# Simple-Robotics/LoIK

Hardware: AMD Instinct MI355X
Metric: IK solves/sec to 1e-6 residual, Talos humanoid, batch=65536 per GPU (higher is better)
Workload: dtype f64

## Files before the change

### loik_amd/csrc/loik_device.hpp

```cpp
#pragma once

#include <hip/hip_runtime.h>

namespace loikb {

constexpr int WAVE = 64;

enum : int {
  JP_CS = 0,
  JP_V = 1,
  JP_F = 4,
  JP_G = 7,
  JP_WZ = 10,
  JP_NUS = 11,
  JP_P = 12,
  JP_R = 15,
  JP_LBUB = 16,
  JP_UD = 17,
  JREC = 20,
  JP_NPERSIST = 12,
  CP_Y = 0,
  CP_ATY = 3,
  CP_B = 6,
  CP_ATB = 9,
// ... 1589 lines not shown
        }
    }
    for (int i = 0; i < 6; ++i) {
      T a = T(0);
      for (int k = 0; k < 6; ++k) a += Al[6 * k + i] * bl[k];
      *elem_ptr<T>(crec, CP_ATB + i / 2, i & 1) = a;
    }
  }
  *elem_ptr<T>(srec, SP_BI, 0) = bn;
}

template <typename T>
__global__ void k_edit_constraints(char* tiles, Layout L, int c_lo, int c_hi, int shift, int B)
{
  const int b = blockIdx.x * blockDim.x + threadIdx.x;
  if (b >= B) return;
  char* lp = lane_ptr<T>(tiles, L, b);
  for (int c = c_lo; c < c_hi; ++c) {
    char* dst = lp + (size_t)(L.off_c + c * L.crec) * pair_bytes<T>();
    const char* src = dst + (size_t)L.crec * pair_bytes<T>();
    const bool copy = shift && c + 1 < c_hi;
    for (int k = 0; k < L.crec; ++k)
      for (int h = 0; h < 2; ++h) *elem_ptr<T>(dst, k, h) = copy ? *elem_ptr<T>(const_cast<char*>(src), k, h) : T(0);
  }
}

enum : int {
  RS_DATA_COLD = 1,
  RS_RECURSION = 2,
  RS_SOLVER = 4,
  RS_Y = 8,
  RS_HCACHE = 16,
  RS_MU = 32,
};
template <typename T>
__device__ __forceinline__ void reset_tile(char* tiles, const Layout& L, int what, T mu0, int tile, int lane)
{
  char* lp = tiles + (size_t)tile * L.tile_pairs * pair_bytes<T>() + (size_t)lane * 2 * sizeof(T);
  if (what & (RS_DATA_COLD | RS_RECURSION)) {
    for (int j = 0; j < L.nb; ++j) {
      char* rec = lp + (size_t)j * JREC * pair_bytes<T>();
      for (int p = JP_V; p < JP_WZ; ++p) stp<T>(rec, p, T(0), T(0));
      stp<T>(rec, JP_WZ, T(0), T(0));
      if (what & RS_DATA_COLD) st_lo<T>(rec, JP_NUS, T(0));
    }
  }
  if (what & (RS_RECURSION | RS_Y)) {
    for (int c = 0; c < L.nc; ++c) {
      char* crec = lp + (size_t)(L.off_c + c * L.crec) * pair_bytes<T>();
      for (int p = CP_Y; p < CP_B; ++p) stp<T>(crec, p, T(0), T(0));
    }
  }
  char* srec = lp + (size_t)L.off_s * pair_bytes<T>();
  if (what & RS_SOLVER) {
    stp<T>(srec, SP_MU, mu0, T(0));
    st_hi<T>(srec, SP_BI, T(0));
    stp<T>(srec, SP_ST, T(0), T(0));
    for (int p = SP_SCAL; p < SREC; ++p) stp<T>(srec, p, T(0), T(0));
  }
  if (what & RS_SOLVER) stp<T>(srec, SP_FLIP, T(0), T(0));
  if (what & RS_MU) stp<T>(srec, SP_MU, mu0, T(0));
  if (what & RS_HCACHE) stp<T>(srec, SP_TAG, T(-1), T(0));
}
template <typename T>
__global__ void __launch_bounds__(WAVE) k_reset(char* tiles, Layout L, int what, T mu0)
{
  reset_tile<T>(tiles, L, what, mu0, (int)blockIdx.x, (int)threadIdx.x);
}

struct MovePlan {
  char* src;
  char* dst_live;
// ... 51 lines not shown
```

### loik_amd/csrc/loik_flat.hpp

```cpp
#pragma once

#include "loik_lean.hpp"

namespace loikb {

constexpr int FLAT_RED = 8;
constexpr int FLAT_PART = 8;
constexpr int FLAT_JMP = 5;
constexpr int FLAT_MAXA = 16;
constexpr int FOLDW = 10;
constexpr int FLAT_COUNTERS_SLOT_HITS = 12;
constexpr int FLAT_NA_SMALL = 10;
constexpr int FSLOT_ROWS = 8;

struct FlatLane {
  int depth;
  int size;
  int jmp[FLAT_JMP];
  int anc[FLAT_MAXA];
  int red[FLAT_RED];
  int helper;
  int part[FLAT_PART];
};

enum : int { FC_LANE = 0, FC_B = 1, FC_Y = 7, FC_ATY = 13, FC_ATYW = 19, FC_ATBW = 25, FC_DY = 31, FC_DLT = 37, FC_ATYF = 43, FC_AW = 49, FC_A = 85,
              FC_VC = FC_DLT , FCD = 121 };
enum : int { FI_BNORM = 0, FI_TGIN, FI_STY, FI_TOLP, FI_TOLD, FI_DYQP, FI_ATDY, FI_UBP, FI_LBM, FI_C1, FI_C2, FI_PRIMAL, FI_DUAL, FI_DX,
             FI_DZ, FI_MULAST, FI_RED , FISC = FI_RED + 16 };

template <int NA>
__host__ __device__ constexpr int flat_xregion()
{
  int n = XROWS * 9;
  if (NA * WAVE + 2 > n) n = NA * WAVE + 2;
  if (WAVE * FOLDW > n) n = WAVE * FOLDW;
  return (n + 1) & ~1;
}
template <int NA> __host__ __device__ constexpr int flat_off_wl() { return flat_xregion<NA>(); }
template <int NA> __host__ __device__ constexpr int flat_off_nbuf() { return flat_off_wl<NA>() + 2 * (NA + 1) * WAVE; }
template <int NA> __host__ __device__ constexpr int flat_off_pbuf() { return flat_off_nbuf<NA>() + WAVE + 2; }
template <int NA> __host__ __device__ constexpr int flat_off_rbuf() { return flat_off_pbuf<NA>() + WAVE + 2; }
template <int NA> __host__ __device__ constexpr int flat_off_tail() { return flat_off_rbuf<NA>() + WAVE; }

template <typename T, int NA>
__host__ __device__ __forceinline__ size_t flat_lds_bytes(int nc, int G, bool a_shared, bool has_hv)
// ... 979 lines not shown
        }
      }
      tail_sync();
      if (on) {
        const T mu = mutab[dsl];
        const T mu_eq = P.mu_scale * mu, mu_in = mu;
        if (cslot >= 0) {
          const T* at = ata_l + (sub * L.nc + cslot) * 21;
#pragma unroll
          for (int k = 0; k < 21; ++k) hh[k] += mu_eq * at[k];
        }
        T U[6], UD[6];
        symv(hh, Sw, U);
        const T dinv = T(1) / (dot6_halves(Sw, U) + mu_in);
#pragma unroll
        for (int k = 0; k < 6; ++k) UD[k] = U[k] * dinv;
#pragma unroll
        for (int k = 0; k < 6; ++k) fslots[fslotA_at(sidx, ndec, dsl, frows, G, k, jlane)] = UD[k];
        fslots[fslotA_at(sidx, ndec, dsl, frows, G, 6, jlane)] = dinv;
        if (has_parent) {
          T* x = xch + lane * HX;
#pragma unroll
          for (int a = 0; a < 6; ++a)
#pragma unroll
            for (int b2 = a; b2 < 6; ++b2) x[sym(a, b2)] = hh[sym(a, b2)] - UD[a] * U[b2];
        }
      }
      tail_sync();
    }
  }
  lb[NA * WAVE + lane] = T(0);
  __builtin_amdgcn_s_waitcnt(0);
  tail_sync();
  for (int dsl = dw0; dsl < dw0 + nw; ++dsl) {
    T UDw[6], dinv = T(0);
#pragma unroll
    for (int k = 0; k < 6; ++k) UDw[k] = isj ? fslots[fslotA_at(sidx, ndec, dsl, frows, G, k, jlane)] : T(0);
    if (isj) dinv = fslots[fslotA_at(sidx, ndec, dsl, frows, G, 6, jlane)];
    T Lc[NA], Wc[NA];
#pragma unroll
    for (int k = 0; k < NA; ++k) {
      Lc[k] = dot6_halves(swt + arow[k] * 6, UDw);
      Wc[k] = T(0);
    }
    tail_sync();
#pragma unroll
    for (int k = 0; k < NA; ++k) lb[k * WAVE + lane] = Lc[k];
    tail_sync();
#pragma unroll
    for (int k = NA - 1; k >= 0; --k) {
      T acc = Lc[k];
#pragma unroll
      for (int k2 = k + 1; k2 < NA; ++k2) acc += lb[k * WAVE + arow[k2]] * Wc[k2];
      Wc[k] = (k < depth - 1) ? -acc : T(0);
    }
    tail_sync();
    if (isj) {
      const size_t base = fslotW_at(sidx, ndec, dsl, frows, fcol);
#pragma unroll
      for (int k = 0; k < NA; ++k)
        if (k < depth - 1) fslots[base + k] = Wc[k];
      fslots[base + depth - 1] = dinv;
    }
  }
}

template <typename T>
__global__ void k_rebuild_ud(char* tiles, Layout L, const JointDesc* __restrict__ jd, const T* __restrict__ uni, T rho, T mu_scale,
                             const T* __restrict__ href_tab, int a_shared, int B, T* __restrict__ scratch)
{
  const int b = blockIdx.x * blockDim.x + threadIdx.x;
  if (b >= B) return;
  char* lp = lane_ptr<T>(tiles, L, b);
  char* srec = lp + (size_t)L.off_s * pair_bytes<T>();
  if (*elem_ptr<T>(srec, SP_TAG, 0) != T(-2)) return;
  const T mu = *elem_ptr<T>(srec, SP_ST, 1);
  const T mu_eq = mu_scale * mu, mu_in = mu;
  T* o = scratch + (size_t)b * L.nb * 21;
  for (int i = 1; i <= L.nb; ++i) {
    for (int r = 0; r < 6; ++r)
      for (int c = r; c < 6; ++c)
        o[(i - 1) * 21 + sym(r, c)] = (jd[i].flags & JF_MASSLESS) ? T(0) : ((r == c ? rho : T(0)) + href_tab[(size_t)i * HREF_ROW + 6 * r + c]);
    if (jd[i].cslot >= 0) {
      const int cs = jd[i].cslot;
      for (int k = 0; k < 21; ++k) {
        const T a = a_shared ? uni[L.nc * 36 + cs * 21 + k]
                             : *elem_ptr<T>(lp + (size_t)(L.off_c + cs * L.crec) * pair_bytes<T>(), CP_ATA + k / 2, k & 1);
        o[(i - 1) * 21 + k] += mu_eq * a;
      }
    }
  }
  for (int i = L.nb; i >= 1; --i) {
    const JointDesc d = jd[i];
    T hh[21], U[6], UD[6], R[9], t[3], part[21];
    for (int k = 0; k < 21; ++k) hh[k] = o[(i - 1) * 21 + k];
// ... 36 lines not shown
```

### loik_amd/csrc/loik_host.hip

```cpp
#include "loik_device.hpp"
#include "loik_tail.hpp"
#include "loik_lean.hpp"
#include "loik_flat.hpp"
#include "loik_flat2.hpp"
#include "loik_passes.hpp"
#include "loik_pose.hpp"
#include "loik_pose_tasks.hpp"
#include "loik_pose_multistart.hpp"
#include "loik_pose_path.hpp"
#include "loik_pose_track.hpp"
#include "loik_pose_accel.hpp"
#include "loik_pose_step.hpp"
#include "loik_flat_inst.hpp"
#ifdef LOIKB_FLAT_SEPARATE_TU
LOIKB_FLAT2_INSTANCES(LOIKB_FLAT2_DECL)
LOIKB_FLAT1_INSTANCES(LOIKB_FLAT1_DECL)
#ifdef LOIKB_TAIL_PROF
int loikb_flat_prof_read(unsigned long long* out, int which, int reset);
#endif
#endif

#include "../../include/loik_amd.h"
#include "../../include/loik_amd_pose.h"
#include "../../include/loik_amd_limits.h"
// ... 213 lines not shown
    int* d_order = nullptr;
    unsigned int* d_order_bins = nullptr;
    int order_n = 0;
    unsigned long long order_epoch = 0;
    int order_holdoff = 0;
    int arrival_n = 0;
    double arrival_ms = 0.0;
    int* d_ring = nullptr;
    int ring_cap = 0;
    void* d_hslots = nullptr;
    size_t hslots_bytes = 0;
    void* d_fslots = nullptr;
    size_t fslots_bytes = 0;
    void* d_park = nullptr;
    unsigned int* d_fmask = nullptr;
    size_t fmask_n = 0;
    void** d_aux = nullptr;
    const void* aux_h[4] = {nullptr, nullptr, nullptr, nullptr};
    size_t park_bytes = 0;
    std::vector<int> h_wave;
    loikb_stats stats{};
    bool unfinished_counted = false;
    bool queue_ready = false;
    bool small_finished = false;
    int rc = 0;
    std::string err;
    std::vector<std::pair<float, float>> solve_iv, tail_iv;
  };
  std::vector<Chunk> chunks;
  hipEvent_t ev_fork = nullptr;
  loikb_stats stats{};
  bool pass_active = false;
  bool zero_state = false;
  unsigned long long inputs_epoch = 1;
  bool href_known = false;
  bool tab_bcast = false;
  double tab_H[36] = {0}, tab_v[6] = {0};
  int log_truncated = 0;
  PassLayout PL{};
  double* d_pass = nullptr;
  int* d_pass_cslot = nullptr;
  int seen_lo = 1 << 20, seen_hi = -(1 << 20);
  unsigned long long end_hist[32] = {0}, end_hist_n = 0;
  unsigned long long solve_serial = 0, end_hist_epoch = 0;
  double* d_log = nullptr;
  int* d_log_rows = nullptr;
  int log_rows_cap = 0;
  bool have_log = false;
  struct PoseState {
    double* d_tgt = nullptr;
    double* d_b = nullptr;
    double* d_err = nullptr;
    double* d_A = nullptr;
    int* d_status = nullptr;
    int* d_steps = nullptr;
    int* d_clink = nullptr;
    unsigned int* d_count = nullptr;
    int nc = 0;
    double timing[4] = {0, 0, 0, 0};
    bool have_limits = false;
    bool flags_valid = false;
    std::vector<PoseLimit> lim;
    PoseLimit* d_lim = nullptr;
    int* d_lflags = nullptr;
    unsigned char* d_inrange = nullptr;
    double2* d_box = nullptr;
// ... 1451 lines not shown
         !(S->opt.flags & (LOIKB_OPT_NO_COMPACTION | LOIKB_OPT_NO_H_CACHE)) && n <= tail_max && S->tune.direct_tail;
}

static bool bushy_goes_on_chip(const loikb_solver_impl* S)
{
  return direct_tail_of(S, S->B, std::max(1, batch_tail_max(S)));
}

template <typename T>
struct TailCtx {
  loikb_solver_impl* S; Chunk* C; Params<T>& P; Bufs<T> Bf;
  loikb_solver_impl::Set& A; int cur, n_cur;
  bool whole_set, small_flat;
  int G, ipw;
  int ndec, kexp_lo;
  const int* list; int n;
  double total_ms = 0.0;
  unsigned long long iters = 0;
};

struct OrderUse { bool ordered = false, was_stale = false; };

static int take_up_order(const loikb_solver_impl* S, Chunk* C, bool eligible, bool count_down, int n_cur, OrderUse* use)
{
  use->ordered = eligible && order_usable(S, C, n_cur);
  use->was_stale = use->ordered && C->order_epoch != S->inputs_epoch;
  if (count_down && C->order_holdoff > 0) --C->order_holdoff;
  if (use->ordered) HIPCHK(hipMemcpyAsync(C->d_slots, C->d_order, sizeof(int) * (size_t)n_cur, hipMemcpyDeviceToDevice, C->stream));
  C->stats.flat_ordered += use->ordered ? 1 : 0;
  return LOIKB_OK;
}

template <typename T>
static int leave_order(const loikb_solver_impl* S, Chunk* C, const loikb_solver_impl::Set& A, int n_cur, bool flat_engine)
{
  HIPCHK(hipMemsetAsync(C->d_order_bins, 0, sizeof(unsigned int) * 2 * ORDER_BINS, C->stream));
  hipLaunchKernelGGL(k_order_count<T>, grid1(n_cur), dim3(256), 0, C->stream, A.tiles, S->L, n_cur, S->opt.max_iter, C->d_order_bins,
                     flat_engine ? C->d_counters + ORDER_DEC_HIST : (unsigned int*)nullptr);
  if (flat_engine) HIPCHK(hipMemcpyAsync(C->h_counters, C->d_counters, NCOUNTERS * sizeof(unsigned int), hipMemcpyDeviceToHost, C->stream));
  hipLaunchKernelGGL(k_order_scan, dim3(1), dim3(ORDER_BINS), 0, C->stream, C->d_order_bins);
  hipLaunchKernelGGL(k_order_scatter<T>, grid1(n_cur), dim3(256), 0, C->stream, A.tiles, S->L, n_cur, S->opt.max_iter, C->d_order_bins, C->d_order);
  HIPCHK(hipGetLastError());
  C->order_n = n_cur;
  C->order_epoch = S->inputs_epoch;
  return LOIKB_OK;
}

static void judge_order(const loikb_solver_impl* S, Chunk* C, int n_cur, OrderUse use, double ms)
{
  if (C->arrival_n != n_cur) { C->arrival_n = n_cur; C->arrival_ms = 0.0; }
  if (!use.ordered) C->arrival_ms = ms;
  else if (use.was_stale && C->arrival_ms > 0.0 && ms > 0.985 * C->arrival_ms) C->order_holdoff = S->tune.flat_order_holdoff;
}

static void record_decades(loikb_solver_impl* S, unsigned int seen, int kexp_lo, unsigned int escaped)
{
  for (int d = 0; d < 16; ++d)
    if (seen & (1u << d)) { S->seen_lo = std::min(S->seen_lo, kexp_lo + d); S->seen_hi = std::max(S->seen_hi, kexp_lo + d); }
  if (escaped) { S->seen_lo = S->plan.kexp_lo; S->seen_hi = S->plan.kexp_lo + S->plan.ndec - 1; }
}

struct FlatLaunch {
  FlatKind kind; int nanc, frows, has_hv; bool small_na;
  int mur;
  int ndec, kexp_lo, dw0, nw;
  int slice;
  double cu_sh; dim3 grid;
};

static int flat_launch_slice(const loikb_solver_impl* S, const Chunk* C, FlatKind kind, int mur, int n, int n_cur, bool ordered)
{
  if (kind == FlatKind::Flat) return 0;
  if (kind == FlatKind::Flat1) return mur == 1 ? 0 : flat_slice_for(S, n, ordered);
  int q = flat_slice_for(S, n, ordered);
  if (q > 0 && (C->d_park == nullptr || (size_t)n_cur * flat2_park_stride(S->nc, true) * sizeof(double) > C->park_bytes)) q = 0;
  if (mur == 1 && S->tune.flat_slice < 0) q = 0;
  return q;
}

static void flat_table_window(const loikb_solver_impl* S, FlatLaunch& F, int n)
{
  int wlo = 0, whi = -1;
  const bool win_ok = F.slice > 0;
  if (S->tune.flat_win_n > 0) { wlo = S->tune.flat_win_lo; whi = wlo + S->tune.flat_win_n - 1; }
  else if (S->tune.flat_build == 2 && win_ok && S->end_hist_n > 0) {
    unsigned long long cum = 0;
    int k03 = 99, k97 = 99;
    for (int k = 0; k < 32; ++k) {
      cum += S->end_hist[k];
      if (k03 == 99 && cum * 100 >= 3ull * S->end_hist_n) k03 = k - 16;
      if (k97 == 99 && cum * 100 >= 97ull * S->end_hist_n) k97 = k - 16;
    }
    wlo = std::min(0, k03); whi = std::max(0, k97);
  }
// ... 97 lines not shown
  if (one_per_wave(F.kind) && X.whole_set && n_first == n_cur) judge_order(S, C, n_cur, use, (double)ms - (double)hms);
  if (S->tune.trace)
    fprintf(stderr, "[loikb] flat engine: %6d instances on %u workgroups, done at %8.3f ms (slots %6.3f ms)  "
                    "inst-iters %9u  wave-iters %7u  slot loads %7u (+ %u served from LDS)  escaped %u  still iterating %u\n",
            n_first, F.grid.x, ms, hms, C->h_counters[1], C->h_counters[5], C->h_counters[6],
            C->h_counters[FLAT_COUNTERS_SLOT_HITS], escaped, C->h_counters[3]);
  C->stats.lean_escaped += (int)escaped;
  C->tail_iv.emplace_back(t0, t0 + ms);
  X.total_ms = ms; X.n = (int)C->h_counters[3]; X.list = next;
  if (X.n == 0 && X.whole_set && X.cur == 0 && n_first == n_cur && S->chunks.size() == 1) { C->stats.n_unfinished = (int)C->h_counters[4]; C->unfinished_counted = true; C->small_finished = small_finish; }
  return LOIKB_OK;
}

template <typename T>
static int launch_flat(TailCtx<T>& X)
{
  loikb_solver_impl* S = X.S; Chunk* C = X.C;
  Params<T>& P = X.P;
  const int n = X.n, n_cur = X.n_cur;
  const bool small_flat = X.small_flat, whole_set = X.whole_set;
  FlatLaunch F;
  F.kind = flat_kind(S); F.nanc = S->flat.nanc; F.small_na = F.nanc <= FLAT_NA_SMALL; F.has_hv = S->Hv_inf_norm != 0.0;
  F.frows = S->flat.fblk;
  F.cu_sh = std::max(1.0, S->ncu * ((double)C->B / (double)S->B));
  F.ndec = X.ndec; F.kexp_lo = X.kexp_lo; F.dw0 = 0;
  const bool can_build2 = S->tune.flat_build && F.kind == FlatKind::Flat2 && C->d_fmask != nullptr && !S->opt.logging && !S->per_link && href_is_scalar(S);
  F.mur = flat_any_mu(S) ? 1 : (can_build2 ? 2 : 0);
  if (F.mur == 1) { F.ndec = 1; F.kexp_lo = 0; }
  if (F.mur == 2) { F.ndec = S->plan.ndec; F.kexp_lo = S->plan.kexp_lo; }
  const size_t need = (size_t)n_cur * F.ndec * F.frows * sizeof(T);
  if (need > C->fslots_bytes) { g_last_error = "internal: decade-slot buffer of the flat engine smaller than the chunk"; return LOIKB_ERR_STATE; }
  P.max_launch_iters = S->opt.max_iter + 1;
  const int mode_keep = P.mode;
  if (whole_set && S->zero_state && S->tune.flat_zero_state) P.mode |= MODE_ZERO_STATE;
  const bool queue_ready = small_flat && C->queue_ready && n_cur == S->B;
  C->queue_ready = false;
  if (!queue_ready && small_flat) hipLaunchKernelGGL(k_queue_init_iota, grid1(std::max(C->ring_cap, NCOUNTERS)), dim3(256), 0, C->stream, C->d_ring, C->ring_cap, C->d_slots, n_cur, C->d_counters, NCOUNTERS);
  else if (!queue_ready) HIPCHK(hipMemsetAsync(C->d_counters, 0, NCOUNTERS * sizeof(unsigned int), C->stream));
  if (!queue_ready) HIPCHK(hipEventRecord(C->ev_k0, C->stream));
  OrderUse use;
  int rc = take_up_order(S, C, !small_flat && whole_set && X.list == C->d_slots && n == n_cur && one_per_wave(F.kind), true, n_cur, &use);
  if (rc) return rc;
  F.slice = flat_launch_slice(S, C, F.kind, F.mur, n, n_cur, use.ordered);
  F.nw = F.ndec;
  if (F.mur == 2) flat_table_window(S, F, n);
  if (F.mur == 0) { F.ndec = X.ndec; F.kexp_lo = X.kexp_lo; F.nw = F.ndec; F.dw0 = 0; }
  if (F.ndec > 0) {
    const dim3 hgrid((unsigned)((n + X.ipw - 1) / X.ipw));
    const size_t slds = (std::max((size_t)(WAVE + 1) * 22, (size_t)((F.small_na ? FLAT_NA_SMALL : FLAT_MAXA) + 1) * WAVE) + (size_t)(WAVE + 1) * 6 +
                         (size_t)X.ipw * S->nc * 21 + 16) * sizeof(T);
    auto* fslots = F.small_na ? k_fslots<T, FLAT_NA_SMALL> : k_fslots<T, FLAT_MAXA>;
    hipLaunchKernelGGL(fslots, hgrid, dim3(WAVE), slds, C->stream, P, X.Bf, (const JointDesc*)S->d_jd, (const TailTopo*)S->d_topo,
                       (const int*)S->d_child_list, (const FlatLane*)S->flat.d_lanes, S->maxdepth, F.nanc, F.frows, S->flat.njmp, X.list, n,
                       X.G, (T*)C->d_fslots, F.kexp_lo, F.ndec, F.dw0, F.nw, F.mur == 2 ? C->d_fmask : (unsigned int*)nullptr);
    HIPCHK(hipGetLastError());
  }
  if (!small_flat) HIPCHK(hipEventRecord(C->ev_k2, C->stream));
  if (!small_flat) hipLaunchKernelGGL(k_ring_fill, grid1(C->ring_cap), dim3(256), 0, C->stream, C->d_ring, C->ring_cap, X.list, n, C->d_counters);
  if ((rc = launch_flat_kernel(X, F))) return rc;
  P.mode = mode_keep;
  int* next = (X.list == C->d_slots) ? C->d_slots2 : C->d_slots;
  const bool small_finish = small_flat && S->tune.small_finish;
  if (small_finish)
    hipLaunchKernelGGL(k_small_finish<T>, dim3(1), dim3(256), 0, C->stream, X.A.tiles, S->L, X.list, n, next, C->d_counters, NCOUNTERS, C->h_counters);
  else
    hipLaunchKernelGGL(k_list_unfinished<T>, grid1(n), dim3(256), 0, C->stream, X.A.tiles, S->L, X.list, n, next, C->d_counters + 3);
  HIPCHK(hipGetLastError());
  C->stats.launches++; C->stats.tail_launches++; C->stats.lean_launches++; C->stats.flat_launches++;
  if (F.kind == FlatKind::Flat2) C->stats.flat_split_launches++;
  HIPCHK(hipEventRecord(C->ev_k1, C->stream));
  const bool order_pass = !small_flat && S->tune.flat_order && whole_set && n == n_cur && one_per_wave(F.kind) && !(S->opt.flags & LOIKB_OPT_FIXED_ITERS);
  if (!order_pass && !small_finish) HIPCHK(hipMemcpyAsync(C->h_counters, C->d_counters, NCOUNTERS * sizeof(unsigned int), hipMemcpyDeviceToHost, C->stream));
  if (order_pass && (rc = leave_order<T>(S, C, X.A, n_cur, true))) return rc;
  HIPCHK(hipStreamSynchronize(C->stream));
  return flat_read_back(X, F, use, order_pass, small_finish, queue_ready, next);
}

template <typename T>
static int launch_lean(TailCtx<T>& X)
{
  loikb_solver_impl* S = X.S; Chunk* C = X.C;
  Params<T>& P = X.P;
  const Bufs<T>& Bf = X.Bf;
  const int n = X.n, n_cur = X.n_cur, G = X.G, ipw = X.ipw, ndec = X.ndec, kexp_lo = X.kexp_lo;
  const int* list = X.list;
  const bool whole_set = X.whole_set, per_link = S->per_link;
  const size_t need = (size_t)n_cur * ndec * HSLOT_PAIRS * G * 2 * sizeof(T);
  if (need > C->hslots_bytes) { g_last_error = "internal: decade-slot buffer smaller than the chunk"; return LOIKB_ERR_STATE; }
  const int waves_cu = S->plan.lean_waves_cu;
  const int ltw = S->plan.lean_wg_waves;
  const size_t lds = ltw * lean_lds_bytes<T>(S->nc, G, S->a_shared);
  if (lds > 64 * 1024) {
    HIPCHK(hipFuncSetAttribute((const void*)k_lean<T, true>, hipFuncAttributeMaxDynamicSharedMemorySize, (int)lds));
    HIPCHK(hipFuncSetAttribute((const void*)k_lean<T, false>, hipFuncAttributeMaxDynamicSharedMemorySize, (int)lds));
    HIPCHK(hipFuncSetAttribute((const void*)k_lean<T, false, true>, hipFuncAttributeMaxDynamicSharedMemorySize, (int)lds));
  }
  const int wg_per_cu = S->tune.lean_wg_per_cu > 0 ? S->tune.lean_wg_per_cu : waves_cu / ltw;
  const int wg_cap = wg_per_cu * std::max(1, (int)(S->ncu * ((double)C->B / (double)S->B) + 0.5));
  HIPCHK(hipEventRecord(C->ev_k0, C->stream));
  OrderUse use;
  int rc = take_up_order(S, C, whole_set && list == C->d_slots && n == n_cur, whole_set, n_cur, &use);
  if (rc) return rc;
  P.max_launch_iters = S->opt.max_iter + 1;
  const int wg_needed = (n + ipw * ltw - 1) / (ipw * ltw);
  const dim3 grid((unsigned)std::min(wg_needed, wg_cap));
  HIPCHK(hipMemsetAsync(C->d_counters, 0, NCOUNTERS * sizeof(unsigned int), C->stream));
// ... 93 lines not shown
  if (whole_set && !small_flat) {
    hipLaunchKernelGGL(k_list_iota, grid1(n_cur), dim3(256), 0, C->stream, C->d_slots, n_cur);
  } else if (!whole_set) {
    C->h_wave.resize(2 * (size_t)nw + 2);
    int* cnt = C->h_wave.data();
    int* off = cnt + nw + 1;
    HIPCHK(hipMemcpyAsync(cnt, A.wave_live, sizeof(int) * nw, hipMemcpyDeviceToHost, C->stream));
    HIPCHK(hipStreamSynchronize(C->stream));
    int total = 0;
    for (int w = 0; w < nw; ++w) { off[w] = total; total += cnt[w]; }
    if (total != n_live) { g_last_error = "tail: live count mismatch"; return LOIKB_ERR_STATE; }
    HIPCHK(hipMemcpyAsync(A.wave_off, off, sizeof(int) * nw, hipMemcpyHostToDevice, C->stream));
    hipLaunchKernelGGL(k_list_live<T>, dim3(nw), dim3(WAVE), 0, C->stream, A.tiles, S->L, n_cur, A.wave_off, C->d_slots);
  }
  HIPCHK(hipGetLastError());
  const int G = lanes_per_instance(S);
  TailCtx<T> X{S, C, P, make_bufs<T>(S, C, cur), A, cur, n_cur, whole_set, small_flat, G, WAVE / G, S->plan.ndec, S->plan.kexp_lo, C->d_slots, n_live};
  P.B = n_cur;
  int tw = S->tune.tail_waves;
  while (tw > 1 && tw * tail_lds_bytes<T>(S->nc, G) > 160 * 1024) --tw;
  const size_t lds = tw * tail_lds_bytes<T>(S->nc, G);
  if (lds > 160 * 1024) { g_last_error = "tail kernel: constraint data exceeds the LDS of a CU"; return LOIKB_ERR_ARG; }
  if (lds > 64 * 1024) {
    HIPCHK(hipFuncSetAttribute((const void*)k_tail<T, true>, hipFuncAttributeMaxDynamicSharedMemorySize, (int)lds));
    HIPCHK(hipFuncSetAttribute((const void*)k_tail<T, false>, hipFuncAttributeMaxDynamicSharedMemorySize, (int)lds));
  }
  if (S->tune.lean_adapt && S->seen_hi >= S->seen_lo && !(S->opt.flags & LOIKB_OPT_FIXED_ITERS) && !S->opt.logging) {
    const int lo = std::max(X.kexp_lo, S->seen_lo - 1), hi = std::min(X.kexp_lo + X.ndec - 1, S->seen_hi + 1);
    if (hi >= lo) { X.kexp_lo = lo; X.ndec = hi - lo + 1; }
  }
  int rc = LOIKB_OK;
  bool engine_ran = true;
  if (flat_here && X.n >= (flat_1pw ? std::max(1, S->tune.flat_min_batch) : 64)) rc = launch_flat(X);
  else if (S->plan.lean && (P.mode & MODE_CACHE_H) && X.n >= 64) rc = launch_lean(X);
  else engine_ran = false;
  if (rc) return rc;
  if (!(engine_ran && X.n == 0) && (rc = launch_tail_kernel(X, tw, lds))) return rc;
  *ms_out = X.total_ms;
  *iters_out = X.iters;
  return LOIKB_OK;
}

template <typename T>
int run_chunk(loikb_solver_impl* S, Chunk* C)
{
  Params<T> P = make_params<T>(S);
  C->stats = loikb_stats{};
  C->unfinished_counted = false;
  C->small_finished = false;
  C->solve_iv.clear();
  C->tail_iv.clear();
  double kernel_ms = 0.0;
  const int max_total = S->opt.max_iter + 1;
  const bool can_compact = !(S->opt.flags & LOIKB_OPT_NO_COMPACTION) && !(S->opt.flags & LOIKB_OPT_FIXED_ITERS);
  const int compact_min = S->opt.compact_min_instances > 0 ? S->opt.compact_min_instances : 64 * WAVE;
  const double compact_ratio = S->tune.compact_ratio;
  const bool use_tail = can_compact && S->nb <= WAVE && S->opt.tail_max_instances >= 0;
  const double share = (double)C->B / (double)S->B;
  const int tail_max = std::max(1, (int)(batch_tail_max(S) * share));
  const bool trace = S->tune.trace;
  const int team_max = S->tune.team_max;
  auto edge_entries = [](const loikb_solver_impl::TeamSched& sc) {
    return std::max(std::max(sc.nslots, 1) * EDGE_ENT, sc.nw > 1 ? sc.nw * Norms<T>::NALL : 0);
  };
  auto lds_bytes = [&](const loikb_solver_impl::TeamSched& sc) {
    return (size_t)(edge_entries(sc) + std::max(sc.nvslots, 1) * 6) * WAVE * sizeof(T);
  };
  constexpr size_t LDS_CU = 160 * 1024, LDS_DEFAULT = 64 * 1024;
  const bool team_ok = S->sched[1].nw > 1 && lds_bytes(S->sched[1]) <= LDS_CU &&
                       5 * (S->sched[1].T_up + S->sched[1].T_down) <= 4 * (S->sched[0].T_up + S->sched[0].T_down);
  if (S->plan.solve_ok) {
    const size_t need = std::max(lds_bytes(S->sched[0]), team_ok ? lds_bytes(S->sched[1]) : (size_t)0);
    if (need > LDS_DEFAULT) {
      HIPCHK(hipFuncSetAttribute((const void*)k_solve<T, true, true>, hipFuncAttributeMaxDynamicSharedMemorySize, (int)need));
      HIPCHK(hipFuncSetAttribute((const void*)k_solve<T, false, true>, hipFuncAttributeMaxDynamicSharedMemorySize, (int)need));
      HIPCHK(hipFuncSetAttribute((const void*)k_solve<T, true, false>, hipFuncAttributeMaxDynamicSharedMemorySize, (int)need));
      HIPCHK(hipFuncSetAttribute((const void*)k_solve<T, false, false>, hipFuncAttributeMaxDynamicSharedMemorySize, (int)need));
    }
  }
  int cur = 0, n_cur = C->B;
  int done_iters = 0;
  unsigned long long inst_iters = 0;
  unsigned int n_live = 0;
  const bool direct_tail = direct_tail_of(S, C->B, tail_max);
  if (!S->plan.solve_ok && !direct_tail) {
    g_last_error = "internal: a tree too bushy for k_solve's LDS slots reached the streaming engine"; return LOIKB_ERR_STATE;
  }
  if (direct_tail) {
    double tms = 0.0;
    unsigned long long tit = 0;
    int rc = run_tail<T>(S, C, P, 0, C->B, C->B, &tms, &tit, true);
    if (rc) return rc;
    kernel_ms += tms;
    if (trace) fprintf(stderr, "[loikb] tail kernel from the first iteration: %d instances  %8.3f ms  inst-iters %9llu\n", C->B, tms, tit);
    C->stats.tail_ms = tms;
    C->stats.tail_instances = C->B;
    C->stats.tail_instance_iterations = tit;
    inst_iters = tit;
  }
  while (!direct_tail) {
    const int tiles_cur = (n_cur + WAVE - 1) / WAVE;
    const bool latency_bound = S->opt.compact_min_instances <= 0 && tiles_cur * (int)S->chunks.size() <= S->ncu;
    const bool may_compact_later = can_compact && n_cur > compact_min && !latency_bound;
    const int lat_iters = S->tune.lat_iters;
    int launch_iters = S->opt.max_launch_iters > 0 ? S->opt.max_launch_iters
                       : (may_compact_later ? 8 : (use_tail || (can_compact && n_cur > compact_min)) ? lat_iters : max_total);
    if (launch_iters > max_total - done_iters) launch_iters = max_total - done_iters;
    P.B = n_cur;
    P.max_launch_iters = launch_iters;
    Bufs<T> Bf = make_bufs<T>(S, C, cur);
    const loikb_solver_impl::TeamSched& sc = S->sched[(team_ok && n_cur <= team_max) ? 1 : 0];
    C->stats.team = sc.nw;
    const int edge_ent = edge_entries(sc);
    const Team tm{sc.d_up, sc.d_down, sc.d_rlist, sc.T_up, sc.T_down, edge_ent};
    const size_t lds = lds_bytes(sc);
    const dim3 grid((unsigned)((n_cur + WAVE - 1) / WAVE)), block(WAVE * sc.nw);
    HIPCHK(hipMemsetAsync(C->d_counters, 0, NCOUNTERS * sizeof(unsigned int), C->stream));
    HIPCHK(hipEventRecord(C->ev_k0, C->stream));
    if (sc.nw > 1) {
// ... 513 lines not shown
{
  if (!S || !H_refs || !v_refs) return LOIKB_ERR_ARG;
  if (!S->have_problem) { g_last_error = "UpdateReferences() before SolveInit()"; return LOIKB_ERR_STATE; }
  if (n != S->ext_nj) { g_last_error = "'H_refs', 'v_refs' have wrong size (one entry per joint incl. the universe)"; return LOIKB_ERR_REFS_SIZE; }
  for (int e = 1; e < n; ++e)
    if (!symmetric6(H_refs + 36 * e)) { g_last_error = "H_refs[i] must be symmetric"; return LOIKB_ERR_HREF_NOT_SYMMETRIC; }
  HIPCHK(hipSetDevice(S->device));
  HIPCHK(hipStreamSynchronize(S->stream));
  ++S->inputs_epoch;
  fill_href_tab(S, H_refs, v_refs, 36, 6);
  S->tab_bcast = false;
  S->href_diag = true;
  for (int e = 0; e < n; ++e) {
    const double *He = H_refs + 36 * e, *ve = v_refs + 6 * e;
    for (int i = 0; i < 6; ++i) {
      double a = 0.0;
      for (int k = 0; k < 6; ++k) {
        a += He[6 * i + k] * ve[k];
        if (e > 0 && i != k && He[6 * i + k] != 0.0) S->href_diag = false;
      }
      if (std::fabs(a) > S->Hv_inf_norm) S->Hv_inf_norm = std::fabs(a);
    }
  }
  S->per_link = true;
  S->pass_active = false;
  int rc;
  if ((rc = upload_href_tab(S))) return rc;
  if ((rc = ensure_hslots(S))) return rc;
  return reset_home(S, RS_HCACHE);
}

static int run_logged(loikb_solver_impl* S, int redo_reset = 0);

int loikb_solve(loikb_solver* S)
{
  if (!S) return LOIKB_ERR_ARG;
  if (!S->have_problem) { g_last_error = "Solve() before SolveInit()"; return LOIKB_ERR_STATE; }
  HIPCHK(hipSetDevice(S->device));
  int rc;
  if ((rc = reset_home(S, RS_RECURSION | RS_SOLVER, !S->opt.logging))) return rc;
  return S->opt.logging ? run_logged(S, RS_RECURSION | RS_SOLVER) : run_main_loop(S);
}

int loikb_solve_full(loikb_solver* S, const double* q, const double* H_ref, const double* v_ref, const int* c_ids,
                     int nc, const double* Ais, const double* bis, const double* lb, const double* ub, int nbound,
                     int in_flags)
{
  if (!S) return LOIKB_ERR_ARG;
  S->offer_queue = !S->opt.logging;
  int rc = solve_init_impl(S, q, H_ref, v_ref, c_ids, nc, Ais, bis, lb, ub, nbound, in_flags, false);
  S->offer_queue = false;
  if (rc) { for (loikb_solver_impl::Chunk& C : S->chunks) C.queue_ready = false; return rc; }
  rc = S->opt.logging ? run_logged(S, S->opt.warm_start ? 0 : (RS_SOLVER | RS_DATA_COLD | RS_Y | RS_HCACHE)) : run_main_loop(S);
  if (rc) (void)hipStreamSynchronize(S->stream);
  return rc;
}

int loikb_solve_tailored(loikb_solver* S, const double* q, int c_id, const double* Ai, const double* bi, int in_flags)
{
  if (!S || (c_id >= 0 && (!Ai || !bi))) return LOIKB_ERR_ARG;
  if (!S->have_problem) { g_last_error = "tailored Solve() before SolveInit()"; return LOIKB_ERR_STATE; }
  HIPCHK(hipSetDevice(S->device));
  int rc;
  struct Deferred { loikb_solver_impl* S; bool armed; ~Deferred() { if (armed) (void)flush_uni(S); S->defer_sync = false; if (armed) (void)hipStreamSynchronize(S->stream); } } deferred{S, true};
  S->defer_sync = true;
  S->pin_off = 0;
  if ((rc = reset_home(S, RS_SOLVER | (S->opt.warm_start ? 0 : RS_DATA_COLD)))) return rc;
  if (c_id >= 0 && (rc = update_eq_single(S, c_id, Ai, bi, in_flags))) return rc;
  S->offer_queue = !S->opt.logging;
  rc = fwd_pass_init(S, q, in_flags);
  S->offer_queue = false;
  if (rc == LOIKB_OK) rc = flush_uni(S);
  if (rc) { for (loikb_solver_impl::Chunk& C : S->chunks) C.queue_ready = false; return rc; }
  S->defer_sync = false;
// ... 837 lines not shown
```

### loik_amd/csrc/loik_lean.hpp

```cpp
#pragma once

#include "loik_tail.hpp"

namespace loikb {

constexpr int LXS = 14;
constexpr int LXA = 0, LXB = 6;
constexpr int LHS = 21;
constexpr int HSLOT_PAIRS = 11;
enum : int { IS_MU = 0, IS_KEXP, IS_ITER, IS_STATUS, IS_TAILIT, IS_C1, IS_C2, IS_NFLIP, IS_TOLP, IS_TOLD, IS_DYQP, IS_ATDY,
             IS_UBP, IS_LBM, IS_BNORM, IS_PRIMAL, IS_DUAL, IS_PRT, IS_PRS, IS_DUALV, IS_STF, IS_DX, IS_DZ, IS_DFIS,
             IS_DYIS, IS_DW, IS_DVIS, IS_DNU, IS_AV, IS_NU, IS_HREFV, IS_G, IS_TGIN, IS_STY, IS_MULAST,
             IS_RED , ISC = IS_RED + 12 };

constexpr int LCD = 26, LCA = 36;
constexpr int LEAN_Q_HEAD = 7, LEAN_Q_TAIL = 8, LEAN_Q_REQUEUES = 9, LEAN_Q_RETIRED = 10;
constexpr int LEAN_DECADES_SEEN = 11;
constexpr int NCOUNTERS = 96;
constexpr int ORDER_DEC_HIST = 64;
enum : int { LC_PAD = 0, LC_B = 1, LC_ATB = 7, LC_Y = 13, LC_ATY = 19 };

template <typename T>
#ifdef LOIKB_PLAIN_RECORDS
__device__ __forceinline__ T cld(const char* p) { return *reinterpret_cast<const T*>(p); }
// ... 859 lines not shown
  for (int k = threadIdx.x; k < ncounters; k += blockDim.x)
    host_counters[k] = __hip_atomic_load(counters + k, __ATOMIC_RELAXED, __HIP_MEMORY_SCOPE_AGENT);
}

constexpr int ORDER_BINS = 256;
template <typename T>
__device__ __forceinline__ int order_bin(char* tiles, const Layout& L, int b, int max_iter)
{
  char* sp = lane_ptr<T>(tiles, L, b);
  const int it = (int)ldp<T>(sp + (size_t)L.off_s * pair_bytes<T>(), SP_BI).y;
  const int k = (int)(((long long)it * ORDER_BINS) / (max_iter > 0 ? max_iter : 1));
  return ORDER_BINS - 1 - (k < 0 ? 0 : k > ORDER_BINS - 1 ? ORDER_BINS - 1 : k);
}
template <typename T>
__global__ void __launch_bounds__(256) k_order_count(char* tiles, Layout L, int n, int max_iter, unsigned int* __restrict__ bins,
                                                     unsigned int* __restrict__ dec_hist = nullptr)
{
  __shared__ unsigned int h[ORDER_BINS], hd[32];
  h[threadIdx.x] = 0u;
  if (threadIdx.x < 32) hd[threadIdx.x] = 0u;
  __syncthreads();
  const int b = blockIdx.x * blockDim.x + threadIdx.x;
  if (b < n) {
    atomicAdd(&h[order_bin<T>(tiles, L, b, max_iter)], 1u);
    if (dec_hist != nullptr) {
      const int kx = (int)ldp<T>(lane_ptr<T>(tiles, L, b) + (size_t)L.off_s * pair_bytes<T>(), SP_MU).y;
      atomicAdd(&hd[kx < -16 ? 0 : kx > 15 ? 31 : kx + 16], 1u);
    }
  }
  __syncthreads();
  if (h[threadIdx.x]) atomicAdd(&bins[threadIdx.x], h[threadIdx.x]);
  if (dec_hist != nullptr && threadIdx.x < 32 && hd[threadIdx.x]) atomicAdd(&dec_hist[threadIdx.x], hd[threadIdx.x]);
}
#ifndef LOIKB_FLAT_KERNELS_TU
__global__ void __launch_bounds__(ORDER_BINS) k_order_scan(unsigned int* __restrict__ bins)
{
  __shared__ unsigned int h[ORDER_BINS];
  const int t = threadIdx.x;
  h[t] = bins[t];
  __syncthreads();
  for (int d = 1; d < ORDER_BINS; d <<= 1) {
    const unsigned int v = t >= d ? h[t - d] : 0u;
    __syncthreads();
    h[t] += v;
    __syncthreads();
  }
  bins[ORDER_BINS + t] = h[t] - bins[t];
}
#endif
template <typename T>
__global__ void __launch_bounds__(256) k_order_scatter(char* tiles, Layout L, int n, int max_iter, unsigned int* __restrict__ bins,
                                                       int* __restrict__ order)
{
  __shared__ unsigned int h[ORDER_BINS], base[ORDER_BINS];
  h[threadIdx.x] = 0u;
  __syncthreads();
  const int b = blockIdx.x * blockDim.x + threadIdx.x;
  int bin = 0;
  unsigned int rank = 0u;
  if (b < n) { bin = order_bin<T>(tiles, L, b, max_iter); rank = atomicAdd(&h[bin], 1u); }
  __syncthreads();
  if (h[threadIdx.x]) base[threadIdx.x] = atomicAdd(&bins[ORDER_BINS + threadIdx.x], h[threadIdx.x]);
  __syncthreads();
  if (b < n) order[base[bin] + rank] = b;
}

// ... 2 lines not shown
```

Measured before the change: 7.091 million.

## Skip joint zeroing on zero-state solves, fuse order count, batch decade slots

```diff
diff --git a/loik_amd/csrc/loik_device.hpp b/loik_amd/csrc/loik_device.hpp
--- a/loik_amd/csrc/loik_device.hpp
+++ b/loik_amd/csrc/loik_device.hpp
@@ -1645,12 +1645,14 @@
   RS_Y = 8,
   RS_HCACHE = 16,
   RS_MU = 32,
+  RS_KEEP_JOINTS = 64,
+  RS_JOINTS = 128,
 };
 template <typename T>
 __device__ __forceinline__ void reset_tile(char* tiles, const Layout& L, int what, T mu0, int tile, int lane)
 {
   char* lp = tiles + (size_t)tile * L.tile_pairs * pair_bytes<T>() + (size_t)lane * 2 * sizeof(T);
-  if (what & (RS_DATA_COLD | RS_RECURSION)) {
+  if ((what & (RS_DATA_COLD | RS_RECURSION | RS_JOINTS)) && !(what & RS_KEEP_JOINTS)) {
     for (int j = 0; j < L.nb; ++j) {
       char* rec = lp + (size_t)j * JREC * pair_bytes<T>();
       for (int p = JP_V; p < JP_WZ; ++p) stp<T>(rec, p, T(0), T(0));
diff --git a/loik_amd/csrc/loik_flat.hpp b/loik_amd/csrc/loik_flat.hpp
--- a/loik_amd/csrc/loik_flat.hpp
+++ b/loik_amd/csrc/loik_flat.hpp
@@ -11,6 +11,10 @@
 constexpr int FOLDW = 10;
 constexpr int FLAT_COUNTERS_SLOT_HITS = 12;
 constexpr int FLAT_NA_SMALL = 10;
+#ifndef LOIKB_FSLOTS_DECADE_GROUP
+#define LOIKB_FSLOTS_DECADE_GROUP 2
+#endif
+constexpr int FSLOTS_DECADE_GROUP = LOIKB_FSLOTS_DECADE_GROUP;
 constexpr int FSLOT_ROWS = 8;
 
 struct FlatLane {
@@ -1056,35 +1060,63 @@
   lb[NA * WAVE + lane] = T(0);
   __builtin_amdgcn_s_waitcnt(0);
   tail_sync();
-  for (int dsl = dw0; dsl < dw0 + nw; ++dsl) {
-    T UDw[6], dinv = T(0);
-#pragma unroll
-    for (int k = 0; k < 6; ++k) UDw[k] = isj ? fslots[fslotA_at(sidx, ndec, dsl, frows, G, k, jlane)] : T(0);
-    if (isj) dinv = fslots[fslotA_at(sidx, ndec, dsl, frows, G, 6, jlane)];
-    T Lc[NA], Wc[NA];
+  constexpr int DG = FSLOTS_DECADE_GROUP;
+  for (int d0 = dw0; d0 < dw0 + nw; d0 += DG) {
+    const int nd = (dw0 + nw - d0 < DG) ? dw0 + nw - d0 : DG;
+    T UDw[DG][6], dinv[DG], Lc[DG][NA];
+#pragma unroll
+    for (int d = 0; d < DG; ++d) {
+      const int dsl = d0 + (d < nd ? d : 0);
+#pragma unroll
+      for (int k = 0; k < 6; ++k) UDw[d][k] = isj ? fslots[fslotA_at(sidx, ndec, dsl, frows, G, k, jlane)] : T(0);
+      dinv[d] = isj ? fslots[fslotA_at(sidx, ndec, dsl, frows, G, 6, jlane)] : T(0);
+    }
+    T swn[6];
+#pragma unroll
+    for (int q = 0; q < 6; ++q) swn[q] = swt[arow[0] * 6 + q];
 #pragma unroll
     for (int k = 0; k < NA; ++k) {
-      Lc[k] = dot6_halves(swt + arow[k] * 6, UDw);
-      Wc[k] = T(0);
-    }
-    tail_sync();
-#pragma unroll
-    for (int k = 0; k < NA; ++k) lb[k * WAVE + lane] = Lc[k];
-    tail_sync();
-#pragma unroll
-    for (int k = NA - 1; k >= 0; --k) {
-      T acc = Lc[k];
-#pragma unroll
-      for (int k2 = k + 1; k2 < NA; ++k2) acc += lb[k * WAVE + arow[k2]] * Wc[k2];
-      Wc[k] = (k < depth - 1) ? -acc : T(0);
-    }
-    tail_sync();
-    if (isj) {
-      const size_t base = fslotW_at(sidx, ndec, dsl, frows, fcol);
-#pragma unroll
-      for (int k = 0; k < NA; ++k)
-        if (k < depth - 1) fslots[base + k] = Wc[k];
-      fslots[base + depth - 1] = dinv;
+      T sw[6];
+#pragma unroll
+      for (int q = 0; q < 6; ++q) sw[q] = swn[q];
+      if (k + 1 < NA) {
+#pragma unroll
+        for (int q = 0; q < 6; ++q) swn[q] = swt[arow[k + 1] * 6 + q];
+      }
+#pragma unroll
+      for (int d = 0; d < DG; ++d) {
+        Lc[d][k] = dot6_halves(sw, UDw[d]);
+        asm volatile("" : "+v"(Lc[d][k]));
+      }
+      __builtin_amdgcn_sched_barrier(0);
+    }
+#pragma unroll
+    for (int d = 0; d < DG; ++d) {
+      if (d >= nd) break;
+      const int dsl = d0 + d;
+      T Wc[NA];
+#pragma unroll
+      for (int k = 0; k < NA; ++k) Wc[k] = T(0);
+      tail_sync();
+#pragma unroll
+      for (int k = 0; k < NA; ++k) lb[k * WAVE + lane] = Lc[d][k];
+      tail_sync();
+#pragma unroll
+      for (int k = NA - 1; k >= 0; --k) {
+        T acc = Lc[d][k];
+#pragma unroll
+        for (int k2 = k + 1; k2 < NA; ++k2) acc += lb[k * WAVE + arow[k2]] * Wc[k2];
+        Wc[k] = (k < depth - 1) ? -acc : T(0);
+      }
+      tail_sync();
+      if (isj) {
+        const size_t base = fslotW_at(sidx, ndec, dsl, frows, fcol);
+#pragma unroll
+        for (int k = 0; k < NA; ++k)
+          if (k < depth - 1) fslots[base + k] = Wc[k];
+        fslots[base + depth - 1] = dinv[d];
+      }
+      __builtin_amdgcn_sched_barrier(0);
     }
   }
 }
diff --git a/loik_amd/csrc/loik_host.hip b/loik_amd/csrc/loik_host.hip
--- a/loik_amd/csrc/loik_host.hip
+++ b/loik_amd/csrc/loik_host.hip
@@ -269,6 +269,7 @@
   loikb_stats stats{};
   bool pass_active = false;
   bool zero_state = false;
+  bool joints_unreset = false;
   unsigned long long inputs_epoch = 1;
   bool href_known = false;
   bool tab_bcast = false;
@@ -1786,11 +1787,13 @@
 }
 
 template <typename T>
-static int leave_order(const loikb_solver_impl* S, Chunk* C, const loikb_solver_impl::Set& A, int n_cur, bool flat_engine)
-{
-  HIPCHK(hipMemsetAsync(C->d_order_bins, 0, sizeof(unsigned int) * 2 * ORDER_BINS, C->stream));
-  hipLaunchKernelGGL(k_order_count<T>, grid1(n_cur), dim3(256), 0, C->stream, A.tiles, S->L, n_cur, S->opt.max_iter, C->d_order_bins,
-                     flat_engine ? C->d_counters + ORDER_DEC_HIST : (unsigned int*)nullptr);
+static int leave_order(const loikb_solver_impl* S, Chunk* C, const loikb_solver_impl::Set& A, int n_cur, bool flat_engine, bool counted = false)
+{
+  if (!counted) {
+    HIPCHK(hipMemsetAsync(C->d_order_bins, 0, sizeof(unsigned int) * 2 * ORDER_BINS, C->stream));
+    hipLaunchKernelGGL(k_order_count<T>, grid1(n_cur), dim3(256), 0, C->stream, A.tiles, S->L, n_cur, S->opt.max_iter, C->d_order_bins,
+                       flat_engine ? C->d_counters + ORDER_DEC_HIST : (unsigned int*)nullptr);
+  }
   if (flat_engine) HIPCHK(hipMemcpyAsync(C->h_counters, C->d_counters, NCOUNTERS * sizeof(unsigned int), hipMemcpyDeviceToHost, C->stream));
   hipLaunchKernelGGL(k_order_scan, dim3(1), dim3(ORDER_BINS), 0, C->stream, C->d_order_bins);
   hipLaunchKernelGGL(k_order_scatter<T>, grid1(n_cur), dim3(256), 0, C->stream, A.tiles, S->L, n_cur, S->opt.max_iter, C->d_order_bins, C->d_order);
@@ -1814,6 +1817,14 @@
   if (escaped) { S->seen_lo = S->plan.kexp_lo; S->seen_hi = S->plan.kexp_lo + S->plan.ndec - 1; }
 }
 
+static bool flat_from_zero_state(const loikb_solver_impl* S, bool whole_set)
+{
+  return whole_set && S->zero_state && S->tune.flat_zero_state;
+}
+static bool flat_honours_zero_state(FlatKind kind, bool sliced)
+{
+  return kind == FlatKind::Flat2 || (kind == FlatKind::Flat1 && !sliced);
+}
 struct FlatLaunch {
   FlatKind kind; int nanc, frows, has_hv; bool small_na;
   int mur;
@@ -1977,11 +1988,13 @@
   if (need > C->fslots_bytes) { g_last_error = "internal: decade-slot buffer of the flat engine smaller than the chunk"; return LOIKB_ERR_STATE; }
   P.max_launch_iters = S->opt.max_iter + 1;
   const int mode_keep = P.mode;
-  if (whole_set && S->zero_state && S->tune.flat_zero_state) P.mode |= MODE_ZERO_STATE;
+  if (flat_from_zero_state(S, whole_set)) P.mode |= MODE_ZERO_STATE;
   const bool queue_ready = small_flat && C->queue_ready && n_cur == S->B;
   C->queue_ready = false;
   if (!queue_ready && small_flat) hipLaunchKernelGGL(k_queue_init_iota, grid1(std::max(C->ring_cap, NCOUNTERS)), dim3(256), 0, C->stream, C->d_ring, C->ring_cap, C->d_slots, n_cur, C->d_counters, NCOUNTERS);
   else if (!queue_ready) HIPCHK(hipMemsetAsync(C->d_counters, 0, NCOUNTERS * sizeof(unsigned int), C->stream));
+  const bool order_pass = !small_flat && S->tune.flat_order && whole_set && n == n_cur && one_per_wave(F.kind) && !(S->opt.flags & LOIKB_OPT_FIXED_ITERS);
+  if (order_pass) HIPCHK(hipMemsetAsync(C->d_order_bins, 0, sizeof(unsigned int) * 2 * ORDER_BINS, C->stream));
   if (!queue_ready) HIPCHK(hipEventRecord(C->ev_k0, C->stream));
   OrderUse use;
   int rc = take_up_order(S, C, !small_flat && whole_set && X.list == C->d_slots && n == n_cur && one_per_wave(F.kind), true, n_cur, &use);
@@ -2002,21 +2015,26 @@
   }
   if (!small_flat) HIPCHK(hipEventRecord(C->ev_k2, C->stream));
   if (!small_flat) hipLaunchKernelGGL(k_ring_fill, grid1(C->ring_cap), dim3(256), 0, C->stream, C->d_ring, C->ring_cap, X.list, n, C->d_counters);
+  if (S->joints_unreset && !((P.mode & MODE_ZERO_STATE) && n == n_cur && flat_honours_zero_state(F.kind, F.slice > 0))) {
+    g_last_error = "internal: the solve's reset left out the joints' state, and its flat launch would fetch it"; return LOIKB_ERR_STATE;
+  }
   if ((rc = launch_flat_kernel(X, F))) return rc;
   P.mode = mode_keep;
   int* next = (X.list == C->d_slots) ? C->d_slots2 : C->d_slots;
   const bool small_finish = small_flat && S->tune.small_finish;
   if (small_finish)
     hipLaunchKernelGGL(k_small_finish<T>, dim3(1), dim3(256), 0, C->stream, X.A.tiles, S->L, X.list, n, next, C->d_counters, NCOUNTERS, C->h_counters);
+  else if (order_pass)
+    hipLaunchKernelGGL(k_list_unfinished_count<T>, grid1(n), dim3(256), 0, C->stream, X.A.tiles, S->L, X.list, n, next, C->d_counters + 3, S->opt.max_iter,
+                       C->d_order_bins, C->d_counters + ORDER_DEC_HIST);
   else
     hipLaunchKernelGGL(k_list_unfinished<T>, grid1(n), dim3(256), 0, C->stream, X.A.tiles, S->L, X.list, n, next, C->d_counters + 3);
   HIPCHK(hipGetLastError());
   C->stats.launches++; C->stats.tail_launches++; C->stats.lean_launches++; C->stats.flat_launches++;
   if (F.kind == FlatKind::Flat2) C->stats.flat_split_launches++;
   HIPCHK(hipEventRecord(C->ev_k1, C->stream));
-  const bool order_pass = !small_flat && S->tune.flat_order && whole_set && n == n_cur && one_per_wave(F.kind) && !(S->opt.flags & LOIKB_OPT_FIXED_ITERS);
   if (!order_pass && !small_finish) HIPCHK(hipMemcpyAsync(C->h_counters, C->d_counters, NCOUNTERS * sizeof(unsigned int), hipMemcpyDeviceToHost, C->stream));
-  if (order_pass && (rc = leave_order<T>(S, C, X.A, n_cur, true))) return rc;
+  if (order_pass && (rc = leave_order<T>(S, C, X.A, n_cur, true, true))) return rc;
   HIPCHK(hipStreamSynchronize(C->stream));
   return flat_read_back(X, F, use, order_pass, small_finish, queue_ready, next);
 }
@@ -2176,6 +2194,7 @@
   int rc = LOIKB_OK;
   bool engine_ran = true;
   if (flat_here && X.n >= (flat_1pw ? std::max(1, S->tune.flat_min_batch) : 64)) rc = launch_flat(X);
+  else if (S->joints_unreset) { g_last_error = "internal: the solve's reset left out the joints' state, and no flat launch takes the batch"; return LOIKB_ERR_STATE; }
   else if (S->plan.lean && (P.mode & MODE_CACHE_H) && X.n >= 64) rc = launch_lean(X);
   else engine_ran = false;
   if (rc) return rc;
@@ -2229,6 +2248,9 @@
   const bool direct_tail = direct_tail_of(S, C->B, tail_max);
   if (!S->plan.solve_ok && !direct_tail) {
     g_last_error = "internal: a tree too bushy for k_solve's LDS slots reached the streaming engine"; return LOIKB_ERR_STATE;
+  }
+  if (!direct_tail && S->joints_unreset) {
+    g_last_error = "internal: the solve's reset left out the joints' state, and the streaming engine would fetch it"; return LOIKB_ERR_STATE;
   }
   if (direct_tail) {
     double tms = 0.0;
@@ -2808,14 +2830,40 @@
 
 static int run_logged(loikb_solver_impl* S, int redo_reset = 0);
 
+static bool solve_skips_joint_zeros(const loikb_solver_impl* S)
+{
+  if (!S->tune.flat_zero_state || S->opt.logging) return false;
+  if (S->opt.mu_update_strat != LOIKB_MU_DEFAULT && S->opt.mu_update_strat != LOIKB_MU_OSQP && S->opt.mu_update_strat != LOIKB_MU_MAXEIGENVALUE) return false;
+  if (!S->plan.solve_ok && !bushy_goes_on_chip(S)) return false;
+  const FlatKind kind = flat_kind(S);
+  if (!one_per_wave(kind) || !flat_applicable(S) || (S->opt.flags & LOIKB_OPT_NO_H_CACHE) || S->chunks.empty()) return false;
+  for (const Chunk& C : S->chunks) {
+    const int tail_max = std::max(1, (int)(batch_tail_max(S) * ((double)C.B / (double)S->B)));
+    if (!direct_tail_of(S, C.B, tail_max) || C.B < std::max(1, S->tune.flat_min_batch)) return false;
+    if (!flat_honours_zero_state(kind, flat_launch_slice(S, &C, kind, flat_any_mu(S) ? 1 : 0, C.B, C.B, false) > 0) ||
+        !flat_honours_zero_state(kind, flat_launch_slice(S, &C, kind, flat_any_mu(S) ? 1 : 0, C.B, C.B, true) > 0)) return false;
+  }
+  return true;
+}
+
 int loikb_solve(loikb_solver* S)
 {
   if (!S) return LOIKB_ERR_ARG;
   if (!S->have_problem) { g_last_error = "Solve() before SolveInit()"; return LOIKB_ERR_STATE; }
   HIPCHK(hipSetDevice(S->device));
   int rc;
-  if ((rc = reset_home(S, RS_RECURSION | RS_SOLVER, !S->opt.logging))) return rc;
-  return S->opt.logging ? run_logged(S, RS_RECURSION | RS_SOLVER) : run_main_loop(S);
+  const bool skip = solve_skips_joint_zeros(S);
+  if ((rc = reset_home(S, RS_RECURSION | RS_SOLVER | (skip ? RS_KEEP_JOINTS : 0), !S->opt.logging))) return rc;
+  if (S->opt.logging) return run_logged(S, RS_RECURSION | RS_SOLVER);
+  S->joints_unreset = skip;
+  rc = run_main_loop(S);
+  S->joints_unreset = false;
+  if (rc && skip) {
+    for (Chunk& C : S->chunks) (void)hipStreamSynchronize(C.stream);
+    (void)reset_home(S, RS_JOINTS);
+    (void)hipStreamSynchronize(S->stream);
+  }
+  return rc;
 }
 
 int loikb_solve_full(loikb_solver* S, const double* q, const double* H_ref, const double* v_ref, const int* c_ids,
diff --git a/loik_amd/csrc/loik_lean.hpp b/loik_amd/csrc/loik_lean.hpp
--- a/loik_amd/csrc/loik_lean.hpp
+++ b/loik_amd/csrc/loik_lean.hpp
@@ -915,6 +915,30 @@
   if (h[threadIdx.x]) atomicAdd(&bins[threadIdx.x], h[threadIdx.x]);
   if (dec_hist != nullptr && threadIdx.x < 32 && hd[threadIdx.x]) atomicAdd(&dec_hist[threadIdx.x], hd[threadIdx.x]);
 }
+template <typename T>
+__global__ void __launch_bounds__(256) k_list_unfinished_count(char* tiles, Layout L, const int* __restrict__ list_in, int n_in, int* __restrict__ list_out,
+                                                               unsigned int* __restrict__ counter, int max_iter, unsigned int* __restrict__ bins,
+                                                               unsigned int* __restrict__ dec_hist)
+{
+  __shared__ unsigned int h[ORDER_BINS], hd[32];
+  h[threadIdx.x] = 0u;
+  if (threadIdx.x < 32) hd[threadIdx.x] = 0u;
+  __syncthreads();
+  const int i = blockIdx.x * blockDim.x + threadIdx.x;
+  if (i < n_in) {
+    const int b = list_in[i];
+    const char* srec = lane_ptr<T>(tiles, L, b) + (size_t)L.off_s * pair_bytes<T>();
+    const int status = (int)ldp<T>(srec, SP_ST).x;
+    const int kx = (int)ldp<T>(srec, SP_MU).y;
+    atomicAdd(&h[order_bin<T>(tiles, L, b, max_iter)], 1u);
+    atomicAdd(&hd[kx < -16 ? 0 : kx > 15 ? 31 : kx + 16], 1u);
+    if (!(status & ST_DONE)) list_out[atomicAdd(counter, 1u)] = b;
+    if (!(status & (ST_CONVERGED | ST_PRIMAL_INF))) atomicAdd(counter + 1, 1u);
+  }
+  __syncthreads();
+  if (h[threadIdx.x]) atomicAdd(&bins[threadIdx.x], h[threadIdx.x]);
+  if (threadIdx.x < 32 && hd[threadIdx.x]) atomicAdd(&dec_hist[threadIdx.x], hd[threadIdx.x]);
+}
 #ifndef LOIKB_FLAT_KERNELS_TU
 __global__ void __launch_bounds__(ORDER_BINS) k_order_scan(unsigned int* __restrict__ bins)
 {
```

After: 7.111 million, median of 3. Within noise of the previous version (+0.3%).
